# d8ahazard/AudioLab

Hardware: AMD Instinct MI355X
Metric: stems*realtime-factor (44.1kHz stereo) (higher is better)
Workload: dtype bf16; 1 GPU; MDX-Net UVR 4-stem (4x TFC-TDF U-Net L=11 g=48 dim_f=3072 dim_t=256 n_fft=6144), 300 s 44.1 kHz stereo in total, margin chunker, windows/launch=52; stems=4

## Files before the change

audiolab_amd/csrc/tdfnet.hip:

```cpp
#include "mma.h"
#include <alsep_gfx950_asm.h>

#include <map>
#include <type_traits>

namespace {

constexpr int kThreads = 256;

template <typename T> struct Vec16;
template <> struct Vec16<float> { static constexpr int N = 4; };
template <> struct Vec16<bf16_t> { static constexpr int N = 8; };
__device__ __forceinline__ void store_vec(float* p, const float* y) { *reinterpret_cast<float4*>(p) = make_float4(y[0], y[1], y[2], y[3]); }
__device__ __forceinline__ void store_vec(bf16_t* p, const float* y) {
    bf16x8 q;
#pragma unroll
    for (int e = 0; e < 8; ++e) q[e] = (bf16_t)y[e];
    *reinterpret_cast<bf16x8*>(p) = q;
}
__device__ __forceinline__ void load_vec(const float* p, float* x) {
    const float4 q = *reinterpret_cast<const float4*>(p);
    x[0] = q.x; x[1] = q.y; x[2] = q.z; x[3] = q.w;
}
__device__ __forceinline__ void load_vec(const bf16_t* p, float* x) {
// ... 1771 lines not shown
#pragma unroll
    for (int j = 0; j < P::D; ++j)
        if (j < nmy) issue(j);
    for (int i = 0; i < nmy; ++i) {
        pipe_wait_tile<P::D, P::ND, P::NS>(i, nmy);
        barrier_nodrain();
        if (i + P::D < nmy) issue(i + P::D);
        if (i > 0) copy_out(i - 1);
        const bf16_t* xs = reinterpret_cast<const bf16_t*>(xring + (size_t)(i % P::NSX) * P::x_bytes);
        f32x4 acc[P::MT][P::NI];
#pragma unroll
        for (int mt = 0; mt < P::MT; ++mt)
#pragma unroll
            for (int ni = 0; ni < P::NI; ++ni) acc[mt][ni] = f32x4{0.f, 0.f, 0.f, 0.f};
        bf16x8 xf[2][P::NI];
        static_for<P::NI>([&](auto nic) {
            constexpr int ni = decltype(nic)::value;
            lds_read_async_b128<ni * 2 * P::XREG>(xf[0][ni], xs + bk[0] / sizeof(bf16_t));
        });
        static_for<P::KS>([&](auto ksc) {
            constexpr int ks = decltype(ksc)::value, b = ks & 1;
            if constexpr (ks + 1 < P::KS) {
                static_for<P::NI>([&](auto nic) {
                    constexpr int ni = decltype(nic)::value;
                    lds_read_async_b128<ni * 2 * P::XREG>(xf[1 - b][ni], xs + bk[ks + 1] / sizeof(bf16_t));
                });
                lds_wait_n<P::NI>();
            } else {
                lds_wait_n<0>();
                if (P::C % 32 != 0) {
#pragma unroll
                    for (int ni = 0; ni < P::NI; ++ni) xf[b][ni] = klast_ok ? xf[b][ni] : bf16x8{};
                }
            }
#pragma unroll
            for (int mt = 0; mt < P::MT; ++mt)
#pragma unroll
                for (int ni = 0; ni < P::NI; ++ni) mma_step(acc[mt][ni], wf[mt][ks], xf[b][ni]);
        });
        bf16_t* sl = reinterpret_cast<bf16_t*>(sring + (size_t)(i % P::NSS) * P::s_bytes + ebase);
        const float* bnl = bn + 4 * lq;
        auto eoff = [&](int mt) {
            int t = 2 * mt + erot;
            t = t >= P::NG ? t - P::NG : t;
            return t * 8;
        };
        bf16x8 ev[2][P::NI];
        f32x4 scv[2], shv[2];
        auto eread = [&](auto mtc) {
            constexpr int mt = decltype(mtc)::value, eb = mt & 1;
            const bf16_t* p = sl + eoff(mt);
            static_for<P::NI>([&](auto nic) {
                constexpr int ni = decltype(nic)::value;
                lds_read_async_b128<ni * 32 * P::NG * 16>(ev[eb][ni], p);
            });
            lds_read_async_f32x4<0>(scv[eb], bnl + mt * 16);
            lds_read_async_f32x4<P::C2 * 4>(shv[eb], bnl + mt * 16);
        };
        eread(std::integral_constant<int, 0>{});
        static_for<P::MT>([&](auto mtc) {
            constexpr int mt = decltype(mtc)::value, b = mt & 1;
            if constexpr (mt + 1 < P::MT) {
                eread(std::integral_constant<int, mt + 1>{});
                lds_wait_n<P::NI + 2>();
            } else {
                lds_wait_n<0>();
            }
            bf16_t* p = sl + eoff(mt) + (lq & 1) * 4;
            static_for<P::NI>([&](auto nic) {
                constexpr int ni = decltype(nic)::value;
                const bf16x4 sk = (lq & 1) ? __builtin_shufflevector(ev[b][ni], ev[b][ni], 4, 5, 6, 7)
                                           : __builtin_shufflevector(ev[b][ni], ev[b][ni], 0, 1, 2, 3);
                bf16x4 q;
#pragma unroll
                for (int r = 0; r < 4; ++r) q[r] = (bf16_t)(fmaxf(fmaf(acc[mt][ni][r], scv[b][r], shv[b][r]), 0.f) * (float)sk[r]);
                lds_write_async_b64(p + ni * 32 * P::NG * 8, q);
            });
        });
    }
    barrier_nodrain();
    copy_out(nmy - 1);
}

#ifndef ALSEP_F16_TU
#include "tdfnet_f32s.h"
#endif

struct DevBuf {
    void* p = nullptr;
    size_t bytes = 0;
};

struct ConvLayer {
    DevBuf w, scale, shift;
    DevBuf w_big;
    DevBuf w_mq;
    DevBuf w_ac;
    int cin = 0, cout = 0;
    bool dma_path = false;
    int split = 0;
    unsigned* range_flag = nullptr;
};
struct GemmLayer {
    DevBuf w, bias, scale, shift;
    int M = 0, K = 0, Kp = 0, Mp = 0;
    bool has_bias = false;
    bool split = false;
    unsigned* range_flag = nullptr;
    bool dma_path = false;
    DevBuf wfrag;
    DevBuf wwide;
};
struct Block {
    std::vector<ConvLayer> tfc;
    std::vector<GemmLayer> tdf;
};

}

struct alsep_net {
    alsep_ctx* ctx = nullptr;
    alsep_net_config cfg{};
    int n = 0;
    bool split = false;
    DevBuf range_flag;
    std::vector<DevBuf> owned;
    DevBuf first_w, first_scale, first_shift, final_w, final_b, zero_page;
    std::vector<Block> enc, dec;
    Block bott;
    std::vector<GemmLayer> ds, us;
};

namespace {

typedef std::map<std::string, std::vector<float>> TensorMap;

template <typename T> T host_cast(float v);
template <> float host_cast<float>(float v) { return v; }
template <> bf16_t host_cast<bf16_t>(float v) { return (bf16_t)v; }

int upload(alsep_net* net, const void* src, size_t bytes, DevBuf* out) {
    void* d = nullptr;
    if (hipMalloc(&d, bytes ? bytes : 16) != hipSuccess) return alsep_fail(net->ctx, ALSEP_ERR_NOMEM, "hipMalloc(%zu) failed", bytes);
    out->p = d;
    out->bytes = bytes;
    net->owned.push_back(*out);
    if (bytes) ALSEP_HIP(net->ctx, hipMemcpy(d, src, bytes, hipMemcpyHostToDevice));
    return ALSEP_OK;
}

const std::vector<float>* find(const TensorMap& tm, const std::string& name, int64_t numel, alsep_ctx* ctx, bool required = true) {
    auto it = tm.find(name);
    if (it == tm.end()) {
        if (required) alsep_fail(ctx, ALSEP_ERR_ARG, "missing tensor '%s'", name.c_str());
        return nullptr;
    }
    if ((int64_t)it->second.size() != numel) {
        alsep_fail(ctx, ALSEP_ERR_ARG, "tensor '%s' has %zu elements, expected %lld", name.c_str(), it->second.size(), (long long)numel);
        return nullptr;
    }
    return &it->second;
}

template <typename T> struct ConvSel;
template <> struct ConvSel<bf16_t> { static constexpr int KC = 48, BN = 48; };
template <> struct ConvSel<float> { static constexpr int KC = 16, BN = 48; };
template <typename T> struct ConvSel16;
template <> struct ConvSel16<bf16_t> { static constexpr int KC = 16, BN = 16; };
template <> struct ConvSel16<float> { static constexpr int KC = 16, BN = 16; };

template <typename T> bool conv_uses_main(int cin, int cout) {
    return cin % ConvSel<T>::KC == 0 && cout % ConvSel<T>::BN == 0;
}

template <typename T, int KC, int BN>
std::vector<T> pack_conv3x3(const std::vector<float>& w, int cin, int cout) {
    typedef ConvCfg<T, KC, BN, 64> Cf;
    const int nq = cin / KC, nn = cout / BN;
    std::vector<T> out((size_t)nn * nq * BN * Cf::KP, host_cast<T>(0.f));
    for (int j = 0; j < nn; ++j)
        for (int q = 0; q < nq; ++q)
            for (int r = 0; r < BN; ++r)
                for (int grp = 0; grp < Cf::NG; ++grp)
                    for (int e = 0; e < Cf::G; ++e) {
                        const int tap = grp / Cf::CG, cg = grp % Cf::CG;
                        const int ci = q * KC + cg * Cf::G + e, co = j * BN + r;
                        const float v = w[(((size_t)co * cin + ci) * 3 + tap / 3) * 3 + tap % 3];
                        out[(((size_t)j * nq + q) * BN + r) * Cf::KP + grp * Cf::G + e] = host_cast<T>(v);
                    }
    return out;
}

std::vector<bf16_t> pack_conv3x3_dma(const std::vector<float>& w, int cin, int cout) {
    typedef ConvB16<64> Cf;
// ... 99 lines not shown
        }
        if (!rc && c == 144) {
            auto pa = pack_conv3x3_allco<9>(*w, c);
            rc = upload(net, pa.data(), pa.size() * sizeof(bf16_t), &L->w_ac);
        }
        if (!rc && (c == 192 || c == 288)) {
            std::vector<bf16_t> pa;
            const size_t slice = (size_t)96 * c * 9;
            for (int g = 0; g < c / 96; ++g) {
                auto pg = pack_conv3x3_allco<6>(std::vector<float>(w->begin() + g * slice, w->begin() + (g + 1) * slice), c);
                pa.insert(pa.end(), pg.begin(), pg.end());
            }
            rc = upload(net, pa.data(), pa.size() * sizeof(bf16_t), &L->w_ac);
        }
    } else if (conv_uses_main<T>(c, c)) {
        auto pk = pack_conv3x3<T, ConvSel<T>::KC, ConvSel<T>::BN>(*w, c, c);
        rc = upload(net, pk.data(), pk.size() * sizeof(T), &L->w);
    } else {
        auto pk = pack_conv3x3<T, ConvSel16<T>::KC, ConvSel16<T>::BN>(*w, c, c);
        rc = upload(net, pk.data(), pk.size() * sizeof(T), &L->w);
    }
    if (rc) return rc;
    if ((rc = upload(net, sc->data(), c * sizeof(float), &L->scale))) return rc;
    return upload(net, sh->data(), c * sizeof(float), &L->shift);
}

template <typename T>
int make_gemm_weights(alsep_net* net, const std::vector<float>& wmk, int M, int K, GemmLayer* L) {
    typedef GemmCfg<T> Gc;
    L->M = M; L->K = K;
#ifndef ALSEP_F16_TU
    if (!is_bf16<T>() && net->split) {
        L->split = true;
        L->range_flag = (unsigned*)net->range_flag.p;
        const std::vector<hs_t> pk = pack_gemm_split(wmk, M, K, &L->Mp, &L->Kp);
        return upload(net, pk.data(), pk.size() * sizeof(hs_t), &L->w);
    }
#endif
    L->Mp = (int)ceil_div64(M, Gc::BR) * Gc::BR;
    L->Kp = (int)ceil_div64(K, Gc::BK) * Gc::BK;
    std::vector<T> pk((size_t)L->Mp * L->Kp, host_cast<T>(0.f));
    for (int m = 0; m < M; ++m)
        for (int k = 0; k < K; ++k) pk[(size_t)m * L->Kp + k] = host_cast<T>(wmk[(size_t)m * K + k]);
    return upload(net, pk.data(), pk.size() * sizeof(T), &L->w);
}

int make_tdf_dma_weights(alsep_net* net, const std::vector<float>& wmk, int M, int K, GemmLayer* L) {
    typedef TdfB16 Tc;
    L->M = M; L->K = K;
    L->Mp = (int)ceil_div64(M, Tc::BM) * Tc::BM;
    L->Kp = (int)ceil_div64(K, Tc::BK) * Tc::BK;
    L->dma_path = true;
    std::vector<bf16_t> pk((size_t)L->Mp * L->Kp, host_cast<bf16_t>(0.f));
    for (int m = 0; m < M; ++m)
        for (int kt = 0; kt < L->Kp / Tc::BK; ++kt)
            for (int g = 0; g < 8; ++g) {
                const int ks = g >> 2, lq = g & 3, pg = g ^ ((m >> 1) & 7);
                for (int e = 0; e < 8; ++e) {
                    const int k = kt * Tc::BK + ks * 32 + (e < 4 ? 4 * lq + e : 16 + 4 * lq + (e - 4));
                    if (k < K) pk[(size_t)m * L->Kp + kt * Tc::BK + pg * 8 + e] = host_cast<bf16_t>(wmk[(size_t)m * K + k]);
                }
            }
    return upload(net, pk.data(), pk.size() * sizeof(bf16_t), &L->w);
}

int make_tdf_wide_weights(alsep_net* net, const std::vector<float>& wmk, int M, int K, GemmLayer* L) {
    const int KT = (int)ceil_div64(K, 64);
    std::vector<bf16_t> pk((size_t)(M / 48) * KT * 6 * 512, host_cast<bf16_t>(0.f));
    for (int rb = 0; rb < M / 48; ++rb)
        for (int kt = 0; kt < KT; ++kt)
            for (int ks = 0; ks < 2; ++ks)
                for (int mi = 0; mi < 3; ++mi)
                    for (int l = 0; l < 64; ++l)
                        for (int e = 0; e < 8; ++e) {
                            const int lq = l >> 4, m = rb * 48 + mi * 16 + (l & 15);
                            const int k = kt * 64 + ks * 32 + (e < 4 ? 4 * lq + e : 16 + 4 * lq + (e - 4));
                            if (k < K)
                                pk[((((size_t)rb * KT + kt) * 2 + ks) * 3 + mi) * 512 + l * 8 + e] =
                                    host_cast<bf16_t>(wmk[(size_t)m * K + k]);
                        }
    return upload(net, pk.data(), pk.size() * sizeof(bf16_t), &L->wwide);
}

int make_frag_weights(alsep_net* net, const std::vector<float>& wmk, int M, int K, DevBuf* out) {
    const int MT = (M + 15) / 16, KS = (K + 31) / 32;
    std::vector<bf16_t> pk((size_t)MT * KS * 64 * 8, host_cast<bf16_t>(0.f));
    for (int mt = 0; mt < MT; ++mt)
        for (int ks = 0; ks < KS; ++ks)
            for (int l = 0; l < 64; ++l)
                for (int e = 0; e < 8; ++e) {
                    const int m = mt * 16 + (l & 15), k = ks * 32 + (l >> 4) * 8 + e;
                    if (m < M && k < K) pk[(((size_t)mt * KS + ks) * 64 + l) * 8 + e] = host_cast<bf16_t>(wmk[(size_t)m * K + k]);
                }
    return upload(net, pk.data(), pk.size() * sizeof(bf16_t), out);
}

template <typename T>
int make_block(alsep_net* net, const TensorMap& tm, const std::string& p, int c, int f, Block* blk) {
    const alsep_net_config& cfg = net->cfg;
    blk->tfc.resize(cfg.l);
    for (int j = 0; j < cfg.l; ++j) {
        int rc = make_conv<T>(net, tm, p + ".tfc." + std::to_string(j), c, &blk->tfc[j]);
        if (rc) return rc;
    }
    const int n_lin = cfg.bn == 0 ? 1 : 2;
    blk->tdf.resize(n_lin);
    for (int j = 0; j < n_lin; ++j) {
        const int fi = (j == 0) ? f : f / cfg.bn;
        const int fo = (n_lin == 1 || j == 1) ? f : f / cfg.bn;
        const std::string q = p + ".tdf." + std::to_string(j);
        auto w = find(tm, q + ".weight", (int64_t)fo * fi, net->ctx);
        auto sc = find(tm, q + ".scale", c, net->ctx);
        auto sh = find(tm, q + ".shift", c, net->ctx);
        if (!w || !sc || !sh) return ALSEP_ERR_ARG;
        GemmLayer* L = &blk->tdf[j];
        int rc = (is_bf16<T>() && c % 48 == 0) ? make_tdf_dma_weights(net, *w, fo, fi, L)
                                               : make_gemm_weights<T>(net, *w, fo, fi, L);
        if (rc) return rc;
        if (L->dma_path && fo % 192 == 0 && (rc = make_tdf_wide_weights(net, *w, fo, fi, L))) return rc;
        if ((rc = upload(net, sc->data(), c * sizeof(float), &L->scale))) return rc;
        if ((rc = upload(net, sh->data(), c * sizeof(float), &L->shift))) return rc;
        auto bi = find(tm, q + ".bias", fo, net->ctx, false);
        if (tm.count(q + ".bias") && !bi) return ALSEP_ERR_ARG;
        L->has_bias = bi != nullptr;
        if (bi && (rc = upload(net, bi->data(), fo * sizeof(float), &L->bias))) return rc;
    }
    return ALSEP_OK;
}

template <typename T>
int build_net(alsep_net* net, const TensorMap& tm) {
    const alsep_net_config& cfg = net->cfg;
    alsep_ctx* ctx = net->ctx;
    const int g = cfg.g, n = net->n;
    int rc;
    {
        auto w = find(tm, "first_conv.weight", (int64_t)g * 4, ctx);
        auto sc = find(tm, "first_conv.scale", g, ctx);
        auto sh = find(tm, "first_conv.shift", g, ctx);
        if (!w || !sc || !sh) return ALSEP_ERR_ARG;
        if ((rc = upload(net, w->data(), w->size() * 4, &net->first_w))) return rc;
        if ((rc = upload(net, sc->data(), g * 4, &net->first_scale))) return rc;
        if ((rc = upload(net, sh->data(), g * 4, &net->first_shift))) return rc;
        auto fw = find(tm, "final_conv.weight", (int64_t)4 * g, ctx);
        auto fb = find(tm, "final_conv.bias", 4, ctx);
        if (!fw || !fb) return ALSEP_ERR_ARG;
        if ((rc = upload(net, fw->data(), fw->size() * 4, &net->final_w))) return rc;
        if ((rc = upload(net, fb->data(), 16, &net->final_b))) return rc;
        const std::vector<char> zeros(256, 0);
        if ((rc = upload(net, zeros.data(), zeros.size(), &net->zero_page))) return rc;
        if ((rc = upload(net, zeros.data(), 16, &net->range_flag))) return rc;
    }
    net->enc.resize(n); net->dec.resize(n); net->ds.resize(n); net->us.resize(n);
    int c = g, f = cfg.dim_f;
    for (int i = 0; i < n; ++i) {
        if ((rc = make_block<T>(net, tm, "encoding_blocks." + std::to_string(i), c, f, &net->enc[i]))) return rc;
        const int c2 = c + g;
        const std::string p = "ds." + std::to_string(i);
        auto w = find(tm, p + ".weight", (int64_t)c2 * c * 4, ctx);
        auto sc = find(tm, p + ".scale", c2, ctx);
        auto sh = find(tm, p + ".shift", c2, ctx);
        if (!w || !sc || !sh) return ALSEP_ERR_ARG;
        std::vector<float> mk((size_t)c2 * 4 * c);
        for (int co = 0; co < c2; ++co)
            for (int ci = 0; ci < c; ++ci)
                for (int d = 0; d < 4; ++d) mk[(size_t)co * 4 * c + d * c + ci] = (*w)[((size_t)co * c + ci) * 4 + d];
        if ((rc = make_gemm_weights<T>(net, mk, c2, 4 * c, &net->ds[i]))) return rc;
        if (is_bf16<T>() && (c == 48 || c == 96 || c == 144) && (rc = make_frag_weights(net, mk, c2, 4 * c, &net->ds[i].wfrag))) return rc;
        if ((rc = upload(net, sc->data(), c2 * 4, &net->ds[i].scale))) return rc;
        if ((rc = upload(net, sh->data(), c2 * 4, &net->ds[i].shift))) return rc;
        c = c2; f /= 2;
    }
    if ((rc = make_block<T>(net, tm, "bottleneck_block", c, f, &net->bott))) return rc;
    for (int i = 0; i < n; ++i) {
        const int c2 = c - g;
        const std::string p = "us." + std::to_string(i);
        auto w = find(tm, p + ".weight", (int64_t)c * c2 * 4, ctx);
        auto sc = find(tm, p + ".scale", c2, ctx);
        auto sh = find(tm, p + ".shift", c2, ctx);
        if (!w || !sc || !sh) return ALSEP_ERR_ARG;
        std::vector<float> mk((size_t)4 * c2 * c), sc4((size_t)4 * c2), sh4((size_t)4 * c2);
        for (int ci = 0; ci < c; ++ci)
            for (int co = 0; co < c2; ++co)
                for (int d = 0; d < 4; ++d) mk[((size_t)d * c2 + co) * c + ci] = (*w)[((size_t)ci * c2 + co) * 4 + d];
        for (int d = 0; d < 4; ++d)
            for (int co = 0; co < c2; ++co) { sc4[d * c2 + co] = (*sc)[co]; sh4[d * c2 + co] = (*sh)[co]; }
        if ((rc = make_gemm_weights<T>(net, mk, 4 * c2, c, &net->us[i]))) return rc;
        if (is_bf16<T>() && (c == 96 || c == 144 || c == 192) && (rc = make_frag_weights(net, mk, 4 * c2, c, &net->us[i].wfrag))) return rc;
        if ((rc = upload(net, sc4.data(), sc4.size() * 4, &net->us[i].scale))) return rc;
        if ((rc = upload(net, sh4.data(), sh4.size() * 4, &net->us[i].shift))) return rc;
        c = c2; f *= 2;
        if ((rc = make_block<T>(net, tm, "decoding_blocks." + std::to_string(i), c, f, &net->dec[i]))) return rc;
    }
    return ALSEP_OK;
}

void conv_work(ProfScope& prof, const ConvLayer& L, size_t elem_bytes, int64_t B, int Th, int Fw) {
    prof.work(18.0 * (double)L.cin * L.cout * B * Th * Fw, (double)elem_bytes * B * Th * Fw * (L.cin + L.cout));
}

template <typename T, int KC, int BN, int TW>
int launch_conv(alsep_ctx* ctx, const ConvLayer& L, const T* X, T* Y, int64_t B, int Th, int Fw) {
// ... 484 lines not shown
                                           hipFuncAttributeMaxDynamicSharedMemorySize, (int)TdfWide<4>::lds_bytes));
        hipLaunchKernelGGL((tdf_bf16_wide_kernel<4, true, 2, true>), grid, dim3(TdfWide<4>::THREADS), TdfWide<4>::lds_bytes,
                           ctx->stream, X, Y, (const bf16_t*)L.wwide.p, bias, (const float*)L.scale.p, (const float*)L.shift.p, R,
                           L.M, L.K, nunits, C, nyb, fin->w, fin->b, (bf16_t*)fin->out, fin->alpha);
        fin->done = true;
        note_launch(ctx, "tdf_bf16_wide_kernel<res,final>");
    } else if (R && rpf == 0) {
        ALSEP_HIP(ctx, hipFuncSetAttribute((const void*)tdf_bf16_wide_kernel<WM, true, 0>,
                                           hipFuncAttributeMaxDynamicSharedMemorySize, (int)Tc::lds_bytes));
        hipLaunchKernelGGL((tdf_bf16_wide_kernel<WM, true, 0>), grid, dim3(Tc::THREADS), Tc::lds_bytes, ctx->stream, X, Y,
                           (const bf16_t*)L.wwide.p, bias, (const float*)L.scale.p, (const float*)L.shift.p, R, L.M, L.K,
                           nunits, C, nyb, (const float*)nullptr, (const float*)nullptr, (bf16_t*)nullptr, 0.f);
    } else if (R) {
        ALSEP_HIP(ctx, hipFuncSetAttribute((const void*)tdf_bf16_wide_kernel<WM, true>,
                                           hipFuncAttributeMaxDynamicSharedMemorySize, (int)Tc::lds_bytes));
        hipLaunchKernelGGL((tdf_bf16_wide_kernel<WM, true>), grid, dim3(Tc::THREADS), Tc::lds_bytes, ctx->stream, X, Y,
                           (const bf16_t*)L.wwide.p, bias, (const float*)L.scale.p, (const float*)L.shift.p, R, L.M, L.K,
                           nunits, C, nyb, (const float*)nullptr, (const float*)nullptr, (bf16_t*)nullptr, 0.f);
    } else {
        ALSEP_HIP(ctx, hipFuncSetAttribute((const void*)tdf_bf16_wide_kernel<WM, false>,
                                           hipFuncAttributeMaxDynamicSharedMemorySize, (int)Tc::lds_bytes));
        hipLaunchKernelGGL((tdf_bf16_wide_kernel<WM, false>), grid, dim3(Tc::THREADS), Tc::lds_bytes, ctx->stream, X, Y,
                           (const bf16_t*)L.wwide.p, bias, (const float*)L.scale.p, (const float*)L.shift.p, R, L.M, L.K,
                           nunits, C, nyb, (const float*)nullptr, (const float*)nullptr, (bf16_t*)nullptr, 0.f);
    }
    note_launch(ctx, R ? "tdf_bf16_wide_kernel<res>" : "tdf_bf16_wide_kernel<nores>");
    ALSEP_LAUNCH_CHECK(ctx, "tdf_bf16_wide_kernel");
    return ALSEP_OK;
}

int run_tdf_dma(alsep_ctx* ctx, const GemmLayer& L, const bf16_t* X, bf16_t* Y, const bf16_t* R, const bf16_t* zp,
                int64_t BT, int C, FinalFold* fin) {
    typedef TdfB16 Tc;
    const int64_t nunits = BT * (C / Tc::UC);
    if (L.wwide.p && tdf_wide_mode() && L.K % 64 == 0 && nunits % 4 == 0) {
        const int mode = tdf_wide_mode();
        const bool can8 = L.M % 384 == 0;
        const bool use8 = mode == 8 ? can8 : (mode == 4 ? false : (can8 && L.M == 384 && !R));
        return use8 ? launch_tdf_wide<8>(ctx, L, X, Y, R, nunits, C, nullptr) : launch_tdf_wide<4>(ctx, L, X, Y, R, nunits, C, fin);
    }
    const int64_t gx = ceil_div64(nunits, Tc::UN);
    if (gx > 0x7fffffff) return alsep_fail(ctx, ALSEP_ERR_ARG, "tdf: too many column tiles");
    const float* bias = L.has_bias ? (const float*)L.bias.p : nullptr;
    ProfScope prof(ctx, ALSEP_PROF_TDF);
    const dim3 grid((unsigned)gx, L.Mp / Tc::BM);
    if (R)
        hipLaunchKernelGGL((tdf_bf16_kernel<true>), grid, dim3(kThreads), Tc::lds_bytes, ctx->stream, X, Y, (const bf16_t*)L.w.p,
                           bias, (const float*)L.scale.p, (const float*)L.shift.p, R, zp, L.M, L.K, L.Kp, nunits, C);
    else
        hipLaunchKernelGGL((tdf_bf16_kernel<false>), grid, dim3(kThreads), Tc::lds_bytes, ctx->stream, X, Y, (const bf16_t*)L.w.p,
                           bias, (const float*)L.scale.p, (const float*)L.shift.p, R, zp, L.M, L.K, L.Kp, nunits, C);
    ALSEP_LAUNCH_CHECK(ctx, "tdf_bf16_kernel");
    return ALSEP_OK;
}
int run_tdf_dma(alsep_ctx* ctx, const GemmLayer&, const float*, float*, const float*, const float*, int64_t, int, FinalFold*) {
    return alsep_fail(ctx, ALSEP_ERR_STATE, "LDS-DMA TDF path is bf16 only");
}

template <typename T>
int run_tdf(alsep_ctx* ctx, const GemmLayer& L, const T* X, T* Y, const T* R, int64_t BT, int C, const void* zero_page,
            FinalFold* fin = nullptr) {
    typedef GemmCfg<T> Gc;
#ifndef ALSEP_F16_TU
    if (L.split) return run_tdf_split(ctx, L, X, Y, R, BT, C);
#endif
    if (L.dma_path) return run_tdf_dma(ctx, L, X, Y, R, (const T*)zero_page, BT, C, fin);
    const int64_t nunits = BT * (C / 16);
    const int64_t gx = ceil_div64(nunits, 8);
    if (gx > 0x7fffffff) return alsep_fail(ctx, ALSEP_ERR_ARG, "tdf_gemm: too many column tiles");
    const float* bias = L.has_bias ? (const float*)L.bias.p : nullptr;
    ProfScope prof(ctx, ALSEP_PROF_TDF);
    if (R)
        hipLaunchKernelGGL((tdf_gemm_kernel<T, true>), dim3((unsigned)gx, L.Mp / Gc::BR), dim3(kThreads), Gc::lds_bytes,
                           ctx->stream, X, Y, (const T*)L.w.p, bias, (const float*)L.scale.p, (const float*)L.shift.p, R,
                           L.M, L.K, L.Kp, nunits, C);
    else
        hipLaunchKernelGGL((tdf_gemm_kernel<T, false>), dim3((unsigned)gx, L.Mp / Gc::BR), dim3(kThreads), Gc::lds_bytes,
                           ctx->stream, X, Y, (const T*)L.w.p, bias, (const float*)L.scale.p, (const float*)L.shift.p, R,
                           L.M, L.K, L.Kp, nunits, C);
    ALSEP_LAUNCH_CHECK(ctx, "tdf_gemm_kernel");
    return ALSEP_OK;
}

template <typename T>
int run_block(alsep_ctx* ctx, const alsep_net* net, const Block& blk, const T* cur, T* a, T* b, T* h, T* dest,
              int64_t B, int Th, int Fw, int c, FinalFold* fin = nullptr) {
    const T* src = cur;
    T* pp[2] = {a, b};
    int rc;
    const int l = (int)blk.tfc.size();
    for (int j = 0; j < l; ++j) {
        T* dst = pp[j & 1];
        if ((rc = run_conv<T>(ctx, blk.tfc[j], src, dst, B, Th, Fw, net->zero_page.p))) return rc;
        src = dst;
    }
    if (blk.tdf.size() == 2) {
        if ((rc = run_tdf<T>(ctx, blk.tdf[0], src, h, (const T*)nullptr, B * Th, c, net->zero_page.p))) return rc;
        return run_tdf<T>(ctx, blk.tdf[1], h, dest, src, B * Th, c, net->zero_page.p, fin);
    }
    return run_tdf<T>(ctx, blk.tdf[0], src, dest, src, B * Th, c, net->zero_page.p, fin);
}

size_t align256(size_t v) { return (v + 255) & ~(size_t)255; }

struct WsLayout {
    size_t p0, p1, p2, h, total;
    std::vector<size_t> skip;
};

WsLayout ws_layout(const alsep_net* net, int64_t B) {
    const alsep_net_config& cfg = net->cfg;
    const size_t es = cfg.dtype == ALSEP_F32 ? 4 : 2;
    WsLayout w;
    const size_t s0 = align256((size_t)B * cfg.dim_t * cfg.dim_f * cfg.g * es);
    size_t off = 0;
    w.p0 = off; off += s0;
    w.p1 = off; off += s0;
    w.p2 = off; off += s0;
    w.h = off;  off += align256(cfg.bn > 0 ? s0 / cfg.bn : 16);
    int c = cfg.g;
    size_t t = cfg.dim_t, f = cfg.dim_f;
    for (int i = 0; i < net->n; ++i) {
        w.skip.push_back(off);
        off += align256((size_t)B * t * f * c * es);
        c += cfg.g; t /= 2; f /= 2;
    }
    w.total = off;
    return w;
}

struct PcmFront {
    const alsep_plan* plan;
    const float* pcm;
    int64_t ch_stride, chunk_stride;
    int zero_low;
};

template <typename T>
int forward_impl(alsep_ctx* ctx, const alsep_net* net, const T* in, T* out, int64_t B, char* ws, float in_scale,
                 float out_alpha, float out_beta, const PcmFront* front = nullptr) {
    const alsep_net_config& cfg = net->cfg;
    const WsLayout L = ws_layout(net, B);
    T* P[3] = {(T*)(ws + L.p0), (T*)(ws + L.p1), (T*)(ws + L.p2)};
    T* H = (T*)(ws + L.h);
    int Th = cfg.dim_t, Fw = cfg.dim_f, c = cfg.g;
    const int64_t npix0 = B * Th * Fw;
    int rc;
    if (front) {
        if ((rc = ALSEP_TU_NAME(alsep_stft_first_conv)(ctx, front->plan, front->pcm, front->ch_stride, front->chunk_stride, B, P[0],
                                                       (const float*)net->first_w.p, (const float*)net->first_scale.p,
                                                       (const float*)net->first_shift.p, cfg.g, in_scale, front->zero_low)))
            return rc;
    } else {
        ProfScope prof(ctx, ALSEP_PROF_POINTWISE);
        const int ppb = kFirstThreads / (cfg.g / Vec16<T>::N);
        const int64_t nblk = std::min<int64_t>(ceil_div64(npix0, ppb), 256 * 16);
        hipLaunchKernelGGL((first_conv_kernel<T>), dim3((unsigned)nblk), dim3(kFirstThreads), 0,
                           ctx->stream, in, P[0], (const float*)net->first_w.p, (const float*)net->first_scale.p,
                           (const float*)net->first_shift.p, npix0, cfg.g, in_scale);
        ALSEP_LAUNCH_CHECK(ctx, "first_conv_kernel");
    }
    FinalFold fold = {(const float*)net->final_w.p, (const float*)net->final_b.p, out, out_alpha, false};
    FinalFold* const fin = (!std::is_same<T, float>::value && out_beta == 0.f) ? &fold : nullptr;
    int ic = 0;
    for (int i = 0; i < net->n; ++i) {
        T* skip = (T*)(ws + L.skip[i]);
        if ((rc = run_block<T>(ctx, net, net->enc[i], P[ic], P[(ic + 1) % 3], P[(ic + 2) % 3], H, skip, B, Th, Fw, c))) return rc;
        const int Tp = Th / 2, Fp = Fw / 2;
        if ((rc = run_pix<T, PIX_DS>(ctx, net->ds[i], skip, P[ic], (const T*)nullptr, B * Tp * Fp, Tp, Fp, c, c + cfg.g))) return rc;
        Th = Tp; Fw = Fp; c += cfg.g;
    }
    {
        T* dest = P[(ic + 1) % 3];
        if ((rc = run_block<T>(ctx, net, net->bott, P[ic], P[(ic + 2) % 3], P[ic], H, dest, B, Th, Fw, c, net->n == 0 ? fin : nullptr)))
            return rc;
        ic = (ic + 1) % 3;
    }
    for (int i = 0; i < net->n; ++i) {
        const T* skip = (const T*)(ws + L.skip[net->n - 1 - i]);
// ... 142 lines not shown
```

Before: 6609 stems*x_realtime.

## Fuse the two TDF bottleneck GEMMs into one persistent bf16 kernel

Adds a persistent kernel that runs both TDF linear layers (F→F/8 and back, each with bias, BN and ReLU, plus the residual add) for F=768 and F=384 in a single launch. Input tiles are double-buffered in LDS via async global-to-LDS loads, and the hidden activation stays in LDS instead of making a round trip through global memory. Weights are held in registers and pre-packed into a fused fragment layout at load time. Routing is gated by an env var and a minimum item count, so smaller workloads fall back to the two-kernel path. In exchange it uses a large LDS footprint and runs at one block per CU.

```diff
diff --git a/audiolab_amd/csrc/tdfnet.hip b/audiolab_amd/csrc/tdfnet.hip
--- a/audiolab_amd/csrc/tdfnet.hip
+++ b/audiolab_amd/csrc/tdfnet.hip
@@ -1877,6 +1877,211 @@
     copy_out(nmy - 1);
 }
 
+template <int F_>
+struct TdfFused {
+    static constexpr int F = F_, H = F_ / 8, UC = 48, WV = 8, THREADS = 64 * WV;
+    static constexpr int ROWS = 768, NU = ROWS / F_;
+    static constexpr int KS1 = F_ / 32, HM = H / 16;
+    static constexpr int HR = (H + 31) / 32 * 32, KS2 = HR / 32;
+    static constexpr int WR = ROWS / WV, MT2 = WR / 16;
+    static constexpr int ND = WR * UC * (int)sizeof(bf16_t) / 1024;
+    static constexpr int WA = NU * HM;
+    static constexpr int CMAX = 192;
+    static constexpr size_t tile_bytes = (size_t)ROWS * UC * sizeof(bf16_t);
+    static constexpr size_t h_bytes = (size_t)NU * HR * UC * sizeof(bf16_t);
+    static constexpr size_t lds_bytes = 2 * tile_bytes + h_bytes + 4 * CMAX * sizeof(float);
+    static_assert(NU * F_ == ROWS && H % 16 == 0 && WA <= WV && F_ % WR == 0 && ND * 1024 == WR * UC * (int)sizeof(bf16_t) && WR % 32 == 0,
+                  "fused TDF geometry");
+    static_assert(lds_bytes <= 160 * 1024, "LDS of a CU");
+};
+
+#ifdef ALSEP_CPU_EMUL
+template <int OFF>
+static inline void lds_read_async_b64(bf16x4& dst, const bf16_t* lds_ptr) { std::memcpy(&dst, reinterpret_cast<const char*>(lds_ptr) + OFF, 8); }
+#else
+template <int OFF>
+__device__ __forceinline__ void lds_read_async_b64(bf16x4& dst, const bf16_t* lds_ptr) {
+    static_assert(OFF >= 0 && OFF < 65536 && OFF % 8 == 0, "ds offset field");
+    const unsigned addr = (unsigned)(unsigned long long)(__attribute__((address_space(3))) const void*)lds_ptr;
+    asm volatile("ds_read_b64 %0, %1 offset:%2" : "=v"(dst) : "v"(addr), "n"(OFF) : "memory");
+}
+#endif
+
+template <int F_>
+__global__ void __launch_bounds__(TdfFused<F_>::THREADS, 1)
+tdf_bf16_fused_kernel(const bf16_t* __restrict__ X, bf16_t* __restrict__ Y, const bf16_t* __restrict__ W1f,
+                      const bf16_t* __restrict__ W2f, const float* __restrict__ bias1, const float* __restrict__ scale1,
+                      const float* __restrict__ shift1, const float* __restrict__ bias2, const float* __restrict__ scale2,
+                      const float* __restrict__ shift2, int nitems, int C) {
+    typedef TdfFused<F_> P;
+    const int tid = threadIdx.x, lane = tid & 63;
+    const int wave = __builtin_amdgcn_readfirstlane(tid >> 6);
+    const int l15 = lane & 15, lq = lane >> 4;
+    char* tiles = alsep_smem;
+    bf16_t* ht = reinterpret_cast<bf16_t*>(alsep_smem + 2 * P::tile_bytes);
+    float* bnl = reinterpret_cast<float*>(alsep_smem + 2 * P::tile_bytes + P::h_bytes);
+    const int upc = C / P::UC;
+
+    for (int i = tid; i < 4 * C; i += P::THREADS) {
+        const int w = i / C, c = i % C;
+        bnl[w * P::CMAX + c] = (w == 0 ? scale1 : (w == 1 ? shift1 : (w == 2 ? scale2 : shift2)))[c];
+    }
+    if (P::HR > P::H) {
+        constexpr int ZG = (P::HR - P::H) * P::UC / 8;
+        for (int i = tid; i < P::NU * ZG; i += P::THREADS)
+            *reinterpret_cast<bf16x8*>(ht + ((i / ZG) * P::HR + P::H) * P::UC + (i % ZG) * 8) = bf16x8{};
+    }
+
+    const bool wa = wave < P::WA;
+    const int ua = wa ? wave / P::HM : 0, mia = wa ? wave % P::HM : 0;
+    const int ub = (wave * P::WR) / P::F, f0 = (wave * P::WR) % P::F;
+    bf16x8 w1[P::KS1], w2[P::MT2][P::KS2];
+#pragma unroll
+    for (int ks = 0; ks < P::KS1; ++ks)
+        w1[ks] = wa ? *reinterpret_cast<const bf16x8*>(W1f + ((size_t)(mia * P::KS1 + ks) * 64 + lane) * 8) : bf16x8{};
+    float b2[P::MT2];
+#pragma unroll
+    for (int mi = 0; mi < P::MT2; ++mi) {
+#pragma unroll
+        for (int ks = 0; ks < P::KS2; ++ks)
+            w2[mi][ks] = *reinterpret_cast<const bf16x8*>(W2f + ((size_t)((f0 / 16 + mi) * P::KS2 + ks) * 64 + lane) * 8);
+        b2[mi] = bias2 ? bias2[f0 + mi * 16 + l15] : 0.f;
+    }
+    const float b1 = (wa && bias1) ? bias1[mia * 16 + l15] : 0.f;
+
+    unsigned xoff[3];
+#pragma unroll
+    for (int j = 0; j < 3; ++j) {
+        const int within = j * 64 + lane;
+        xoff[j] = (unsigned)(((within / 6) * C + (within % 6) * 8) * (int)sizeof(bf16_t));
+    }
+    const int trow = l15 >> 2, tcol = (l15 & 3) * 4;
+    const unsigned xa_off = (unsigned)(((ua * P::F + 4 * lq + trow) * P::UC + tcol) * (int)sizeof(bf16_t));
+    const bf16_t* hl = ht + (ub * P::HR + 4 * lq + trow) * P::UC + tcol;
+    bf16_t* hw = ht + (ua * P::HR + mia * 16 + l15) * P::UC + 4 * lq;
+    const unsigned eb_off = (unsigned)(((wave * P::WR + l15) * P::UC + 4 * lq) * (int)sizeof(bf16_t));
+    const unsigned co_off = (unsigned)(wave * P::ND * 1024 + lane * 16);
+
+    const int nmy = (nitems - (int)blockIdx.x + (int)gridDim.x - 1) / (int)gridDim.x;
+    auto unit_cb = [&](int i, int u) { return ((((int)blockIdx.x + i * (int)gridDim.x) * P::NU + u) % upc) * P::UC; };
+    auto unit_base = [&](int i, int u) {
+        const int un = ((int)blockIdx.x + i * (int)gridDim.x) * P::NU + u;
+        return ((int64_t)(un / upc) * P::F) * C + (un % upc) * P::UC;
+    };
+    auto issue = [&](int i) {
+        const ALSEP_GLOBAL char* src = opaque_uniform_gptr(reinterpret_cast<const char*>(X + unit_base(i, ub) + (int64_t)f0 * C));
+        char* dst = tiles + (size_t)(i & 1) * P::tile_bytes + (size_t)wave * (P::ND * 1024);
+#pragma unroll
+        for (int q = 0; q < P::ND; ++q) glds16_base(src + (size_t)(q / 3) * 32 * C * sizeof(bf16_t), xoff[q % 3], dst + q * 1024);
+    };
+
+    wait_vmcnt<0>();
+    if (nmy > 0) issue(0);
+    for (int i = 0; i < nmy; ++i) {
+        if (i > 0) wait_vmcnt<P::ND>();
+        else wait_vmcnt<0>();
+        barrier_nodrain();
+        if (i + 1 < nmy) issue(i + 1);
+        char* tile = tiles + (size_t)(i & 1) * P::tile_bytes;
+
+        if (wa) {
+            const bf16_t* xl = reinterpret_cast<const bf16_t*>(tile + xa_off);
+            const bf16_t* xl2 = xl + 12 * 32 * P::UC;
+            f32x4 acc[3];
+#pragma unroll
+            for (int ni = 0; ni < 3; ++ni) acc[ni] = f32x4{0.f, 0.f, 0.f, 0.f};
+            bf16x8 xf[2][3];
+            static_for<3>([&](auto nic) {
+                constexpr int ni = decltype(nic)::value;
+                xf[0][ni] = tdfw_read_frag<ni * 32>(xl);
+            });
+            static_for<P::KS1>([&](auto ksc) {
+                constexpr int ks = decltype(ksc)::value, b = ks & 1;
+                if constexpr (ks + 1 < P::KS1) {
+                    constexpr int k1 = ks + 1;
+                    const bf16_t* bp = k1 >= 12 ? xl2 : xl;
+                    static_for<3>([&](auto nic) {
+                        constexpr int ni = decltype(nic)::value;
+                        xf[1 - b][ni] = tdfw_read_frag<(k1 % 12) * 32 * P::UC * 2 + ni * 32>(bp);
+                    });
+                    lds_read_tr16_wait_n<6>();
+                } else {
+                    lds_read_tr16_wait_n<0>();
+                }
+#pragma unroll
+                for (int ni = 0; ni < 3; ++ni) mma_step(acc[ni], xf[b][ni], w1[ks]);
+            });
+            const float* bp = bnl + unit_cb(i, ua) + 4 * lq;
+            f32x4 sc[3], sh[3];
+            static_for<3>([&](auto nic) {
+                constexpr int ni = decltype(nic)::value;
+                lds_read_async_f32x4<ni * 64>(sc[ni], bp);
+                lds_read_async_f32x4<P::CMAX * 4 + ni * 64>(sh[ni], bp);
+            });
+            lds_wait_n<0>();
+            static_for<3>([&](auto nic) {
+                constexpr int ni = decltype(nic)::value;
+                bf16x4 q;
+#pragma unroll
+                for (int r = 0; r < 4; ++r) q[r] = (bf16_t)fmaxf(fmaf(acc[ni][r] + b1, sc[ni][r], sh[ni][r]), 0.f);
+                lds_write_async_b64(hw + ni * 16, q);
+            });
+        }
+        barrier_nodrain();
+
+        {
+            const float* bp = bnl + 2 * P::CMAX + unit_cb(i, ub) + 4 * lq;
+            bf16_t* el = reinterpret_cast<bf16_t*>(tile + eb_off);
+            static_for<P::MT2>([&](auto mic) {
+                constexpr int mi = decltype(mic)::value;
+                bf16x8 hf[P::KS2][3];
+                static_for<P::KS2 * 3>([&](auto jc) {
+                    constexpr int ks = decltype(jc)::value / 3, ni = decltype(jc)::value % 3;
+                    hf[ks][ni] = tdfw_read_frag<ks * 32 * P::UC * 2 + ni * 32>(hl);
+                });
+                f32x4 acc[3];
+#pragma unroll
+                for (int ni = 0; ni < 3; ++ni) acc[ni] = f32x4{0.f, 0.f, 0.f, 0.f};
+                lds_read_tr16_wait_n<0>();
+#pragma unroll
+                for (int ks = 0; ks < P::KS2; ++ks)
+#pragma unroll
+                    for (int ni = 0; ni < 3; ++ni) mma_step(acc[ni], hf[ks][ni], w2[mi][ks]);
+                bf16x4 xr[3];
+                f32x4 sc[3], sh[3];
+                static_for<3>([&](auto nic) {
+                    constexpr int ni = decltype(nic)::value;
+                    lds_read_async_b64<(mi * 16 * P::UC + ni * 16) * 2>(xr[ni], el);
+                    lds_read_async_f32x4<ni * 64>(sc[ni], bp);
+                    lds_read_async_f32x4<P::CMAX * 4 + ni * 64>(sh[ni], bp);
+                });
+                lds_wait_n<0>();
+                static_for<3>([&](auto nic) {
+                    constexpr int ni = decltype(nic)::value;
+                    bf16x4 q;
+#pragma unroll
+                    for (int r = 0; r < 4; ++r)
+                        q[r] = (bf16_t)(fmaxf(fmaf(acc[ni][r] + b2[mi], sc[ni][r], sh[ni][r]), 0.f) + (float)xr[ni][r]);
+                    lds_write_async_b64(el + mi * 16 * P::UC + ni * 16, q);
+                });
+            });
+            __builtin_amdgcn_wave_barrier();
+            const bf16_t* cl = reinterpret_cast<const bf16_t*>(tile + co_off);
+            bf16x8 q[P::ND];
+            static_for<P::ND>([&](auto tc) {
+                constexpr int t = decltype(tc)::value;
+                lds_read_async_b128<t * 1024>(q[t], cl);
+            });
+            lds_wait_n<0>();
+            ALSEP_GLOBAL char* yb = const_cast<ALSEP_GLOBAL char*>(
+                opaque_uniform_gptr(reinterpret_cast<const char*>(Y + unit_base(i, ub) + (int64_t)f0 * C)));
+#pragma unroll
+            for (int t = 0; t < P::ND; ++t)
+                stream_store(reinterpret_cast<ALSEP_GLOBAL bf16x8*>(yb + (size_t)(t / 3) * 32 * C * sizeof(bf16_t) + xoff[t % 3]), q[t]);
+        }
+    }
+}
+
 #ifndef ALSEP_F16_TU
 #include "tdfnet_f32s.h"
 #endif
@@ -1905,6 +2110,7 @@
     bool dma_path = false;
     DevBuf wfrag;
     DevBuf wwide;
+    DevBuf wfused;
 };
 struct Block {
     std::vector<ConvLayer> tfc;
@@ -2170,6 +2376,20 @@
     return upload(net, pk.data(), pk.size() * sizeof(bf16_t), &L->wwide);
 }
 
+int make_tdf_fused_weights(alsep_net* net, const std::vector<float>& wmk, int M, int K, GemmLayer* L) {
+    const int MT = M / 16, KS = (K + 31) / 32;
+    std::vector<bf16_t> pk((size_t)MT * KS * 512, host_cast<bf16_t>(0.f));
+    for (int mt = 0; mt < MT; ++mt)
+        for (int ks = 0; ks < KS; ++ks)
+            for (int l = 0; l < 64; ++l)
+                for (int e = 0; e < 8; ++e) {
+                    const int lq = l >> 4, m = mt * 16 + (l & 15);
+                    const int k = ks * 32 + (e < 4 ? 4 * lq + e : 16 + 4 * lq + (e - 4));
+                    if (k < K) pk[(((size_t)mt * KS + ks) * 64 + l) * 8 + e] = host_cast<bf16_t>(wmk[(size_t)m * K + k]);
+                }
+    return upload(net, pk.data(), pk.size() * sizeof(bf16_t), &L->wfused);
+}
+
 int make_frag_weights(alsep_net* net, const std::vector<float>& wmk, int M, int K, DevBuf* out) {
     const int MT = (M + 15) / 16, KS = (K + 31) / 32;
     std::vector<bf16_t> pk((size_t)MT * KS * 64 * 8, host_cast<bf16_t>(0.f));
@@ -2206,6 +2426,8 @@
                                                : make_gemm_weights<T>(net, *w, fo, fi, L);
         if (rc) return rc;
         if (L->dma_path && fo % 192 == 0 && (rc = make_tdf_wide_weights(net, *w, fo, fi, L))) return rc;
+        if (L->dma_path && n_lin == 2 && cfg.bn == 8 && (f == 768 || f == 384) && (rc = make_tdf_fused_weights(net, *w, fo, fi, L)))
+            return rc;
         if ((rc = upload(net, sc->data(), c * sizeof(float), &L->scale))) return rc;
         if ((rc = upload(net, sh->data(), c * sizeof(float), &L->shift))) return rc;
         auto bi = find(tm, q + ".bias", fo, net->ctx, false);
@@ -2856,6 +3078,47 @@
     return ALSEP_OK;
 }
 
+enum { kTdfFusedF768 = 1, kTdfFusedF384 = 2 };
+constexpr int kTdfFusedRouted = kTdfFusedF768 | kTdfFusedF384;
+constexpr int64_t kTdfFusedFloor[2] = {9984, 3328};
+int tdf_fused_mode() {
+    static const int v = env_int("ALSEP_TDF_FUSED", 1);
+    return v;
+}
+template <int F_>
+int launch_tdf_fused(alsep_ctx* ctx, const GemmLayer& A, const GemmLayer& B, const bf16_t* X, bf16_t* Y, int64_t nitems, int C) {
+    typedef TdfFused<F_> P;
+    static const int cap = env_int("ALSEP_TDF_FUSED_GRID", 0);
+    int64_t grid = device_cu_count(ctx);
+    if (cap > 0 && cap < grid) grid = cap;
+    if (nitems < grid) grid = nitems;
+    ProfScope prof(ctx, ALSEP_PROF_TDF);
+    ALSEP_HIP(ctx, hipFuncSetAttribute((const void*)tdf_bf16_fused_kernel<F_>, hipFuncAttributeMaxDynamicSharedMemorySize, (int)P::lds_bytes));
+    hipLaunchKernelGGL((tdf_bf16_fused_kernel<F_>), dim3((unsigned)grid), dim3(P::THREADS), P::lds_bytes, ctx->stream, X, Y,
+                       (const bf16_t*)A.wfused.p, (const bf16_t*)B.wfused.p, A.has_bias ? (const float*)A.bias.p : nullptr,
+                       (const float*)A.scale.p, (const float*)A.shift.p, B.has_bias ? (const float*)B.bias.p : nullptr,
+                       (const float*)B.scale.p, (const float*)B.shift.p, (int)nitems, C);
+    note_launch(ctx, "tdf_bf16_kernel");
+    note_launch(ctx, "tdf_bf16_kernel");
+    ALSEP_LAUNCH_CHECK(ctx, "tdf_bf16_fused_kernel");
+    return ALSEP_OK;
+}
+int run_tdf_fused(alsep_ctx* ctx, const Block& blk, const bf16_t* X, bf16_t* Y, int64_t BT, int C, bool* done) {
+    const GemmLayer& A = blk.tdf[0];
+    const GemmLayer& B = blk.tdf[1];
+    const int mode = tdf_fused_mode();
+    if (mode <= 0 || !A.dma_path || !B.dma_path || !A.wfused.p || !B.wfused.p || C % 48 != 0 || C > TdfFused<768>::CMAX) return ALSEP_OK;
+    const bool f768 = B.M == 768;
+    const int64_t nunits = BT * (C / 48);
+    const int nu = f768 ? TdfFused<768>::NU : TdfFused<384>::NU;
+    if (nunits <= 0 || nunits % nu != 0 || nunits > 0x7fffffff) return ALSEP_OK;
+    const int64_t nitems = nunits / nu;
+    if (mode == 1 && (!(kTdfFusedRouted & (f768 ? kTdfFusedF768 : kTdfFusedF384)) || nitems < kTdfFusedFloor[f768 ? 0 : 1])) return ALSEP_OK;
+    *done = true;
+    return f768 ? launch_tdf_fused<768>(ctx, A, B, X, Y, nitems, C) : launch_tdf_fused<384>(ctx, A, B, X, Y, nitems, C);
+}
+int run_tdf_fused(alsep_ctx*, const Block&, const float*, float*, int64_t, int, bool*) { return ALSEP_OK; }
+
 template <typename T>
 int run_block(alsep_ctx* ctx, const alsep_net* net, const Block& blk, const T* cur, T* a, T* b, T* h, T* dest,
               int64_t B, int Th, int Fw, int c, FinalFold* fin = nullptr) {
@@ -2869,6 +3132,8 @@
         src = dst;
     }
     if (blk.tdf.size() == 2) {
+        bool fused = false;
+        if ((rc = run_tdf_fused(ctx, blk, src, dest, B * Th, c, &fused)) || fused) return rc;
         if ((rc = run_tdf<T>(ctx, blk.tdf[0], src, h, (const T*)nullptr, B * Th, c, net->zero_page.p))) return rc;
         return run_tdf<T>(ctx, blk.tdf[1], h, dest, src, B * Th, c, net->zero_page.p, fin);
     }
```

Result: faster. 6699 stems*x_realtime, median of 6 (+1.4%).
